# pranshu-raj-211/dmdqn

Measured on NVIDIA B200. Metric: agent-updates/sec, higher is better.
Workload: dtype f32

## Files before the change

dmdqn_b200/csrc/api.cu:

```cuda
#include <stdarg.h>
#include <string.h>
#include "common.cuh"

namespace dmdqn {

static thread_local char g_error[512] = "";

void set_error(const char* fmt, ...) {
    va_list ap;
    va_start(ap, fmt);
    vsnprintf(g_error, sizeof(g_error), fmt, ap);
    va_end(ap);
}

int validate_dims(const dmdqn_dims* d) {
    DMDQN_CHECK_ARG(d != nullptr, "dims is NULL");
    DMDQN_CHECK_ARG(d->n_agents >= 1, "n_agents=%d must be >= 1", d->n_agents);
    DMDQN_CHECK_ARG(d->n_nets == d->n_agents || d->n_nets == 1,
                    "n_nets=%d must be n_agents (independent) or 1 (shared)", d->n_nets);
    DMDQN_CHECK_ARG(d->obs_dim >= 1 && d->obs_stride >= d->obs_dim && d->obs_stride % 16 == 0 &&
                        d->obs_stride <= 128,
                    "obs_dim=%d obs_stride=%d: stride must be a multiple of 16 in [obs_dim, 128]",
                    d->obs_dim, d->obs_stride);
    DMDQN_CHECK_ARG(d->hidden == 64 || d->hidden == 128 || d->hidden == 256 || d->hidden == 512,
// ... 118 lines not shown
    if (rc) return rc;
    DMDQN_CHECK_ARG(nets && nets->theta && obs && eps && w_explore && w_action && actions_out, "act: NULL argument");
    DMDQN_CHECK_ARG(obs_in_stride >= dims->obs_dim, "obs_in_stride=%d < obs_dim=%d", obs_in_stride, dims->obs_dim);
    return launch_act(*dims, *nets, obs, obs_in_stride, eps, w_explore, w_action, actions_out, q_out, dueling,
                      (cudaStream_t)stream);
}

int dmdqn_act(const dmdqn_dims* dims, const dmdqn_nets* nets, const float* obs, int32_t obs_in_stride,
              const double* eps, const uint32_t* w_explore, const uint32_t* w_action, int32_t* actions_out,
              float* q_out, void* stream) {
    return run_act(dims, nets, obs, obs_in_stride, eps, w_explore, w_action, actions_out, q_out, false, stream);
}

int dmdqn_act_dueling(const dmdqn_dims* dims, const dmdqn_nets* nets, const float* obs, int32_t obs_in_stride,
                      const double* eps, const uint32_t* w_explore, const uint32_t* w_action, int32_t* actions_out,
                      float* q_out, void* stream) {
    return run_act(dims, nets, obs, obs_in_stride, eps, w_explore, w_action, actions_out, q_out, true, stream);
}

int dmdqn_push(const dmdqn_dims* dims, const dmdqn_replay* replay, const float* obs, const int32_t* act,
               const double* rew, const float* next_obs, const uint8_t* done, int32_t in_stride,
               const uint8_t* mask, void* stream) {
    int rc = validate_dims(dims);
    if (rc) return rc;
    DMDQN_CHECK_ARG(replay && replay->obs && replay->next_obs && replay->act && replay->rew && replay->done &&
                        replay->n_written, "push: NULL replay pointer");
    DMDQN_CHECK_ARG(!replay->priority || replay->priority_max, "push: priority is set but priority_max is NULL");
    DMDQN_CHECK_ARG(obs && act && rew && next_obs && done, "push: NULL transition pointer");
    DMDQN_CHECK_ARG(in_stride >= dims->obs_dim, "in_stride=%d < obs_dim=%d", in_stride, dims->obs_dim);
    return launch_push(*dims, *replay, obs, act, rew, next_obs, done, in_stride, mask, (cudaStream_t)stream);
}

static int check_n_step(const dmdqn_hparams* hp) {
    DMDQN_CHECK_ARG(hp->n_step >= 0 && hp->n_step <= DMDQN_MAX_NSTEP, "n_step=%d must be in [0, %d] (0 and 1: one-step targets)",
                    hp->n_step, DMDQN_MAX_NSTEP);
    return DMDQN_OK;
}

static_assert(offsetof(dmdqn_hparams, dueling) == 76 && sizeof(dmdqn_hparams) == 112,
              "dueling sits in the former interior padding of dmdqn_hparams: no other field moves");

static int check_dueling(const dmdqn_hparams* hp) {
    DMDQN_CHECK_ARG(hp->dueling == 0 || hp->dueling == 1, "dueling=%d must be 0 (plain head) or 1 (dueling heads)", hp->dueling);
    return DMDQN_OK;
}

static int check_learn_args(const dmdqn_dims* dims, const dmdqn_hparams* hp, const dmdqn_replay* replay,
                            const dmdqn_nets* nets, const void* draws) {
    DMDQN_CHECK_ARG(hp && replay && nets && draws, "NULL argument");
    if (int rc = check_n_step(hp)) return rc;
    if (int rc = check_dueling(hp)) return rc;
    DMDQN_CHECK_ARG(replay->obs && replay->next_obs && replay->act && replay->rew && replay->done &&
                        replay->n_written, "NULL replay pointer");
    DMDQN_CHECK_ARG(nets->theta && nets->theta_tgt && nets->adam_m && nets->adam_v && nets->learn_step,
                    "NULL network pointer");
    DMDQN_CHECK_ARG(hp->sample_mode >= 0 && hp->sample_mode <= DMDQN_SAMPLE_PRIORITIZED, "sample_mode=%d", hp->sample_mode);
    if (hp->sample_mode == DMDQN_SAMPLE_PRIORITIZED) {
        DMDQN_CHECK_ARG(replay->priority && replay->priority_max,
                        "sample_mode=prioritized needs the replay's priority and priority_max arrays (NULL priority pointer)");
        DMDQN_CHECK_ARG(!(dims->n_nets == 1 && dims->n_agents > 1),
                        "sample_mode=prioritized serves independent networks only (n_nets=%d, n_agents=%d share parameters)",
                        dims->n_nets, dims->n_agents);
    }
    DMDQN_CHECK_ARG(hp->loss == DMDQN_LOSS_MSE || hp->loss == DMDQN_LOSS_HUBER, "loss=%d", hp->loss);
    DMDQN_CHECK_ARG(hp->precision >= DMDQN_PRECISION_FP32 && hp->precision <= DMDQN_PRECISION_TF32X3, "precision=%d",
                    hp->precision);
    return DMDQN_OK;
}

static int run_learn(const dmdqn_dims* dims, const dmdqn_hparams* hp, const dmdqn_replay* replay, const dmdqn_nets* nets,
                     const void* draws, const uint8_t* learn_mask, float* metrics_out, void* workspace,
                     size_t workspace_bytes, int32_t stages, float* grads, int32_t global_batch, void* stream) {
    Workspace w;
    int rc = check_workspace(dims, workspace, workspace_bytes, &w);
    if (rc) return rc;
    rc = check_learn_args(dims, hp, replay, nets, draws);
    if (rc) return rc;
    if (grads) DMDQN_CHECK_ARG(global_batch >= dims->batch, "global_batch=%d < batch=%d", global_batch, dims->batch);
    if (stages & DMDQN_STAGE_SAMPLE) {
        if (hp->dueling) {
            rc = launch_fold(*dims, *nets, (char*)workspace, w, (cudaStream_t)stream);
            if (rc) return rc;
        }
        rc = launch_sample(*dims, *hp, *replay, *nets, draws, learn_mask, 1, (char*)workspace, w, (cudaStream_t)stream);
        if (rc) return rc;
    }
    return launch_learn(*dims, *hp, *replay, *nets, metrics_out, (char*)workspace, w, stages, grads, global_batch,
                        (cudaStream_t)stream);
}

int dmdqn_sample(const dmdqn_dims* dims, const dmdqn_hparams* hp, const dmdqn_replay* replay,
                 const dmdqn_nets* nets, const void* draws, const uint8_t* learn_mask, int32_t advance_step,
                 void* workspace, size_t workspace_bytes, void* stream) {
    Workspace w;
    int rc = check_workspace(dims, workspace, workspace_bytes, &w);
    if (rc) return rc;
    rc = check_learn_args(dims, hp, replay, nets, draws);
    if (rc) return rc;
    return launch_sample(*dims, *hp, *replay, *nets, draws, learn_mask, advance_step, (char*)workspace, w,
                         (cudaStream_t)stream);
}

int dmdqn_gather(const dmdqn_dims* dims, const dmdqn_replay* replay, const void* workspace,
                 size_t workspace_bytes, float* states, int32_t* actions, float* rewards, float* next_states,
                 float* dones, int32_t* active_out, void* stream) {
    Workspace w;
    int rc = check_workspace(dims, const_cast<void*>(workspace), workspace_bytes, &w);
    if (rc) return rc;
    DMDQN_CHECK_ARG(replay && replay->obs && replay->next_obs, "gather: NULL replay pointer");
    DMDQN_CHECK_ARG(states && actions && rewards && next_states && dones, "gather: NULL output");
    return launch_gather(*dims, *replay, (const char*)workspace, w, states, actions, rewards, next_states, dones,
                         active_out, (cudaStream_t)stream);
}

int dmdqn_learn_stages(const dmdqn_dims* dims, const dmdqn_hparams* hp, const dmdqn_replay* replay,
                       const dmdqn_nets* nets, const void* draws, const uint8_t* learn_mask, float* metrics_out,
                       void* workspace, size_t workspace_bytes, int32_t stages, void* stream) {
    return run_learn(dims, hp, replay, nets, draws, learn_mask, metrics_out, workspace, workspace_bytes, stages, nullptr, 0,
                     stream);
}

int dmdqn_learn(const dmdqn_dims* dims, const dmdqn_hparams* hp, const dmdqn_replay* replay,
                const dmdqn_nets* nets, const void* draws, const uint8_t* learn_mask, float* metrics_out,
                void* workspace, size_t workspace_bytes, void* stream) {
    return run_learn(dims, hp, replay, nets, draws, learn_mask, metrics_out, workspace, workspace_bytes, kAllStages, nullptr,
                     0, stream);
}

int dmdqn_step_host(const dmdqn_dims* dims, const dmdqn_hparams* hp, const dmdqn_replay* replay,
                    const dmdqn_nets* nets, const dmdqn_step_block* blk, const void* host_block, void* device_block,
                    float* metrics_dev, float* metrics_host, void* workspace, size_t workspace_bytes, void* stream) {
    int rc = validate_dims(dims);
    if (rc) return rc;
    DMDQN_CHECK_ARG(hp && blk && host_block && device_block && metrics_dev && metrics_host, "step_host: NULL argument");
    rc = check_n_step(hp);
    if (rc) return rc;
    rc = check_dueling(hp);
    if (rc) return rc;
    const size_t offs[6] = {blk->obs_off, blk->next_obs_off, blk->act_off, blk->rew_off, blk->done_off, blk->draws_off};
    for (size_t o : offs) DMDQN_CHECK_ARG(o % 16 == 0 && o < blk->bytes, "step_host: offset %zu is not a multiple of 16 inside the block", o);
    cudaStream_t s = (cudaStream_t)stream;
    char* d = static_cast<char*>(device_block);
    DMDQN_CUDA(cudaMemcpyAsync(d, host_block, blk->bytes, cudaMemcpyHostToDevice, s));
    rc = dmdqn_push(dims, replay, reinterpret_cast<const float*>(d + blk->obs_off), reinterpret_cast<const int32_t*>(d + blk->act_off),
                    reinterpret_cast<const double*>(d + blk->rew_off), reinterpret_cast<const float*>(d + blk->next_obs_off),
                    reinterpret_cast<const uint8_t*>(d + blk->done_off), blk->in_stride, nullptr, stream);
    if (rc) return rc;
    rc = dmdqn_learn(dims, hp, replay, nets, d + blk->draws_off, nullptr, metrics_dev, workspace, workspace_bytes, stream);
    if (rc) return rc;
    DMDQN_CUDA(cudaMemcpyAsync(metrics_host, metrics_dev, (size_t)dims->n_nets * DMDQN_METRICS_STRIDE * sizeof(float),
                               cudaMemcpyDeviceToHost, s));
    return DMDQN_OK;
}

int dmdqn_learn_grads(const dmdqn_dims* dims, const dmdqn_hparams* hp, const dmdqn_replay* replay,
                      const dmdqn_nets* nets, const void* draws, const uint8_t* learn_mask, int32_t global_batch,
                      float* grads_out, float* metrics_out, void* workspace, size_t workspace_bytes, void* stream) {
    DMDQN_CHECK_ARG(grads_out != nullptr, "grads_out is NULL");
    return run_learn(dims, hp, replay, nets, draws, learn_mask, metrics_out, workspace, workspace_bytes, kAllStages,
                     grads_out, global_batch, stream);
}

int dmdqn_adam_apply(const dmdqn_dims* dims, const dmdqn_hparams* hp, const dmdqn_nets* nets, const float* grads,
                     void* workspace, size_t workspace_bytes, void* stream) {
    Workspace w;
    int rc = check_workspace(dims, workspace, workspace_bytes, &w);
    if (rc) return rc;
// ... 239 lines not shown
```

dmdqn_b200/csrc/common.cuh:

```cuda
#pragma once
#include <cuda_runtime.h>
#include <stdint.h>
#include <stdio.h>
#include "../../include/dmdqn_b200.h"

namespace dmdqn {

void set_error(const char* fmt, ...);

#define DMDQN_CHECK_ARG(cond, ...)                                  \
    do {                                                            \
        if (!(cond)) {                                              \
            ::dmdqn::set_error(__VA_ARGS__);                        \
            return DMDQN_ERR_ARG;                                   \
        }                                                           \
    } while (0)

#define DMDQN_CUDA(expr)                                                              \
    do {                                                                              \
        cudaError_t _e = (expr);                                                      \
        if (_e != cudaSuccess) {                                                      \
            ::dmdqn::set_error("%s failed: %s", #expr, cudaGetErrorString(_e));       \
            return DMDQN_ERR_CUDA;                                                    \
        }                                                                             \
// ... 194 lines not shown
    float one_m_b1, one_m_b2, tau;
    int ws_tiles;
    int tc_tiles;
    const int32_t *rows, *nrows, *act_b, *active;
    const float *r_hat, *disc_b;
    const float4* adam_sc;
    float *y, *q_all, *q_next, *tq_all, *h1, *dh1, *dh2;
    float *part_loss, *part_b3, *part_w3, *part_b2, *part_b1;
    uint32_t* mask2;
    float2* ga;
    float* w3_copy;
    int* error;
    float* metrics;
    float* grads;
    int chain;
    int *sched, *k4a_done, *k3_done;
    int per;
    const float* is_w;
    double per_alpha, per_eps;
    const float* head[2];
    int64_t head_stride;
    int dueling;
};
LearnArgs make_learn_args(const dmdqn_dims& d, const dmdqn_hparams& hp, const dmdqn_replay& rp, const dmdqn_nets& nets,
                          char* ws, const Workspace& w, float* metrics, float* grads, int loss_batch);

__device__ __forceinline__ void per_store_priority(const LearnArgs& A, int row, float delta) {
    const float p = (float)pow(fabs((double)delta) + A.per_eps, A.per_alpha);
    if (!isfinite(p)) return;
    A.rp.priority[row] = p;
    atomicMax(reinterpret_cast<int*>(A.rp.priority_max) + row / A.d.capacity, __float_as_int(p));
}

struct AdamStep {
    float alpha, eps, one_m_b1, one_m_b2, tau;
    int sync;
};
__device__ __forceinline__ AdamStep adam_step(const LearnArgs& A, int g) {
    const float4 sc = __ldg(A.adam_sc + g);
    return {sc.x, sc.y, A.one_m_b1, A.one_m_b2, A.tau, __float_as_int(sc.z)};
}

template <typename Load>
__device__ __forceinline__ void finish_metrics(const LearnArgs& A, int g, int tiles, Load ld) {
    double ls = 0, qs = 0, qq = 0, hist[4] = {0, 0, 0, 0};
#pragma unroll 1
    for (int r = 0; r < tiles; ++r) {
        const float* pl = A.part_loss + ((size_t)g * tiles + r) * 8;
        ls += ld(pl); qs += ld(pl + 1); qq += ld(pl + 2);
        for (int a = 0; a < 4; ++a) hist[a] += ld(pl + 3 + a);
    }
    const double cnt = (double)A.d.batch * A.d.n_actions, mean = qs / cnt, var = fmax(qq / cnt - mean * mean, 0.0);
    float* m = A.metrics + g * DMDQN_METRICS_STRIDE;
    m[0] = (float)(ls / A.loss_batch);
    m[1] = (float)mean;
    m[2] = (float)sqrt(var);
    for (int a = 0; a < 4; ++a) m[3 + a] = (float)hist[a];
    m[7] = 1.f;
}

constexpr int kMaxDevices = 64;
int device_sm_count(int* n_sm);
int opt_in_dynamic_smem(const void* kernel, size_t bytes, size_t (&cache)[kMaxDevices]);

int launch_featurize(int32_t n, const int32_t* halting, const int32_t* phase, const double* next_switch,
                     const double* phase_dur, double sim_time, const uint8_t* signal_valid,
                     const int32_t* nbr_idx, const int32_t* phase_lut, const double* snapshot,
                     double lw, double gw, double* own_out, float* obs_out, int32_t obs_out_stride,
                     double* reward_out, double* global_out, int64_t* scratch, cudaStream_t s);
int launch_featurize_alt(int32_t n, const int32_t* halting, const int32_t* phase, const double* next_switch,
                         const uint8_t* signal_valid, double sim_time, const int32_t* nbr_idx, const double* prev_own,
                         double* own_out, float* obs_out, int32_t obs_out_stride, double* reward_out, cudaStream_t s);
int launch_act(const dmdqn_dims& d, const dmdqn_nets& nets, const float* obs, int32_t stride,
               const double* eps, const uint32_t* w1, const uint32_t* w2, int32_t* actions, float* q_out, bool dueling,
               cudaStream_t s, const dmdqn_noisy* noisy = nullptr);
int launch_noisy_fold(const dmdqn_dims& d, bool dueling, const dmdqn_nets& nets, const dmdqn_noisy& nz, cudaStream_t s);
int launch_noisy_adam_apply(const dmdqn_dims& d, const dmdqn_hparams& hp, const dmdqn_nets& nets, const dmdqn_noisy& nz,
                            const float* grads, char* ws, const Workspace& w, cudaStream_t s);
int launch_push(const dmdqn_dims& d, const dmdqn_replay& rp, const float* obs, const int32_t* act,
                const double* rew, const float* next_obs, const uint8_t* done, int32_t in_stride,
                const uint8_t* mask, cudaStream_t s);
int launch_sample(const dmdqn_dims& d, const dmdqn_hparams& hp, const dmdqn_replay& rp, const dmdqn_nets& nets,
                  const void* draws, const uint8_t* learn_mask, int advance, char* ws, const Workspace& w,
                  cudaStream_t s);
int launch_gather(const dmdqn_dims& d, const dmdqn_replay& rp, const char* ws, const Workspace& w,
                  float* states, int32_t* actions, float* rewards, float* next_states, float* dones,
                  int32_t* active_out, cudaStream_t s);
int launch_learn(const dmdqn_dims& d, const dmdqn_hparams& hp, const dmdqn_replay& rp, const dmdqn_nets& nets,
                 float* metrics, char* ws, const Workspace& w, int stages, float* grads, int loss_batch, cudaStream_t s);
bool tc_supported(const dmdqn_dims& d);
int launch_learn_tc(const LearnArgs& A, int precision, int stages, cudaStream_t s);
int launch_adam_apply(const dmdqn_dims& d, const dmdqn_hparams& hp, const dmdqn_nets& nets, const float* grads, char* ws,
                      const Workspace& w, cudaStream_t s);
int launch_clip_adam_apply(const dmdqn_dims& d, const dmdqn_hparams& hp, const dmdqn_nets& nets, const float* grads,
                           double clipnorm, float* norms_out, char* ws, const Workspace& w, cudaStream_t s);
int launch_sync_target(const dmdqn_dims& d, const dmdqn_nets& nets, const uint8_t* mask, double tau, bool dueling,
                       cudaStream_t s);
int launch_fold(const dmdqn_dims& d, const dmdqn_nets& nets, char* ws, const Workspace& w, cudaStream_t s);
int launch_peer_adam(const dmdqn_dims& d, const dmdqn_hparams& hp, const dmdqn_nets& nets, const dmdqn_peers& peers,
                     const float* my_loss_src, float* loss_out, char* ws, const Workspace& w, cudaStream_t s);

}
```

dmdqn_b200/csrc/learn_tc.cu:

```cuda
#include <cuda.h>
#include <string.h>
#include "common.cuh"

namespace dmdqn {

namespace {

constexpr int H = 256;
constexpr int BM = 128;
constexpr int EW = 16;
constexpr int NT = EW * 32;
constexpr int W_MMA = EW, W_TMA = EW + 1, W_CONV = EW + 2;
constexpr int CONV_WARPS = 6, CONV_GROUP_WARPS = 2;
constexpr int NT_F = (EW + 8) * 32;
constexpr int REGS_EPI = 104, REGS_AUX = 32;
constexpr int KC = 16;
constexpr uint32_t ATOM = BM * 128;
constexpr unsigned long long WAIT_LIMIT_NS = 2000000000ull;

__device__ __forceinline__ uint32_t smem_u32(const void* p) { return (uint32_t)__cvta_generic_to_shared(p); }

__device__ __forceinline__ uint64_t make_desc(uint32_t saddr, uint32_t lbo_bytes, uint32_t sbo_bytes, uint32_t layout) {
    return (uint64_t)((saddr >> 4) & 0x3FFF) | (uint64_t)((lbo_bytes >> 4) & 0x3FFF) << 16 |
           (uint64_t)((sbo_bytes >> 4) & 0x3FFF) << 32 | (uint64_t)1 << 46 | (uint64_t)layout << 61;
// ... 924 lines not shown
    th = th - __fdividef(m * k.alpha, sq + k.eps);
}

struct Wg {
    static constexpr int STAGES = 3;
    static constexpr uint32_t A_BYTES = KC * BM * 4;
    static constexpr uint32_t B_BYTES = KC * H * 4;
    static constexpr uint32_t AUX = 2 * A_BYTES + 2 * B_BYTES;
    static constexpr uint32_t AUX_MASK = 128;
    static constexpr uint32_t AUX_BYTES = 6144;
    static constexpr uint32_t STG = AUX + AUX_BYTES;
    static constexpr int TLD = 36;
    static constexpr uint32_t TILES = STAGES * STG;
    static constexpr uint32_t W3T = TILES + 8 * 32 * TLD * 4;
    static constexpr uint32_t BARS = W3T + 2 * 4 * H * 4;
    static constexpr uint32_t FULL = 0, CONV = 24, EMPTY = 48, ACC_FULL = 72, ACC_FREE = 88, TMEM = 104;
    static constexpr int NQ = 8;
    static constexpr uint32_t QFULL = 112, QITEM = QFULL + 8 * NQ;
    static constexpr uint32_t TOTAL = BARS + 256;
    static constexpr int EPI_WARPS = 8, CONV_WARPS = 8;
    static constexpr int NCONV = CONV_WARPS * 32;
    static constexpr int NTW = 20 * 32;
    static constexpr int REGS_EPI = 160, REGS_CONV = 64, REGS_AUX = 32;
};
__device__ __forceinline__ void conv_sync() { asm volatile("bar.sync 1, 256;" ::: "memory"); }

__device__ __forceinline__ void wg_item(int q, int G, int& g, int& t) {
    if (q < 2 * G) { g = q >> 1; t = q & 1; }
    else { g = q - 2 * G; t = 2; }
}

__device__ __forceinline__ int wg_pop(uint32_t bars, int& nq, bool& ok) {
    const uint32_t slot = (uint32_t)nq & (Wg::NQ - 1);
    int q = -1;
    if ((threadIdx.x & 31) == 0) {
        if (ok) ok = mbar_wait(bars + Wg::QFULL + 8 * slot, (uint32_t)(nq >> 3) & 1u);
        if (ok) asm volatile("ld.shared.s32 %0, [%1];" : "=r"(q) : "r"(bars + Wg::QITEM + 4 * slot));
    }
    ++nq;
    q = __shfl_sync(0xffffffffu, q, 0);
    if (q < 0) ok = __shfl_sync(0xffffffffu, (int)ok, 0) != 0;
    return q;
}
__device__ __forceinline__ float ldcg_f(const float* p) {
    float v;
    asm volatile("ld.global.cg.f32 %0, [%1];" : "=f"(v) : "l"(p));
    return v;
}

template <int PASSES>
__global__ void __launch_bounds__(Wg::NTW, 1) tc_wgrad_kernel(const LearnArgs A, const __grid_constant__ CUtensorMap tmap_h1,
                                                              const __grid_constant__ CUtensorMap tmap_dh1) {
    extern __shared__ uint8_t smem_raw[];
    const int B = A.d.batch, Dp = A.d.obs_stride, G = A.d.n_nets;
    const int tid = threadIdx.x, warp = tid >> 5, lane = tid & 31;
    const uint32_t sbase = (smem_u32(smem_raw) + 1023u) & ~1023u;
    const uint32_t bars = sbase + Wg::BARS;
    const int n_items = 3 * G;
    const int nchunks = (B + KC - 1) / KC;

    if (tid == 0) {
        for (int s = 0; s < Wg::STAGES; ++s) {
            mbar_init(bars + Wg::FULL + 8 * s, 1);
            mbar_init(bars + Wg::CONV + 8 * s, Wg::CONV_WARPS);
            mbar_init(bars + Wg::EMPTY + 8 * s, 1);
        }
        for (int b = 0; b < 2; ++b) {
            mbar_init(bars + Wg::ACC_FULL + 8 * b, 1);
            mbar_init(bars + Wg::ACC_FREE + 8 * b, Wg::EPI_WARPS);
        }
        for (int b = 0; b < Wg::NQ; ++b) mbar_init(bars + Wg::QFULL + 8 * b, 1);
        asm volatile("fence.mbarrier_init.release.cluster;" ::: "memory");
    }
    if (warp == 0) {
        asm volatile("tcgen05.alloc.cta_group::1.sync.aligned.shared::cta.b32 [%0], %1;" ::"r"(bars + Wg::TMEM), "r"(512));
        asm volatile("tcgen05.relinquish_alloc_permit.cta_group::1.sync.aligned;" ::);
    }
    tc_fence_before();
    __syncthreads();
    tc_fence_after();
    uint32_t tmem;
    asm volatile("ld.shared.u32 %0, [%1];" : "=r"(tmem) : "r"(bars + Wg::TMEM));
    bool ok = true;

    if (warp >= Wg::EPI_WARPS + Wg::CONV_WARPS) {
        regs_dec<Wg::REGS_AUX>();
        if (warp == Wg::EPI_WARPS + Wg::CONV_WARPS) {
            {
                uint32_t used = 0;
                int n = 0, nq = 0;
                for (;;) {
                    const int q = wg_pop(bars, nq, ok);
                    if (q < 0) break;
                    if (lane != 0) continue;
                    int g, t;
                    wg_item(q, G, g, t);
                    const bool is_w2 = t < 2;
                    const uint32_t acc_buf = (uint32_t)(n & 1);
                    const uint32_t d_tmem = tmem + acc_buf * 256u;
                    const uint32_t idesc = make_idesc(!is_w2, is_w2);
                    if (n >= 2 && ok)
                        ok = mbar_wait(bars + Wg::ACC_FREE + 8 * acc_buf, (uint32_t)((n >> 1) - 1) & 1u);
                    for (int c = 0; c < nchunks; ++c) {
                        const uint32_t s = used % Wg::STAGES, u = used / Wg::STAGES;
                        if (ok) ok = mbar_wait(bars + Wg::CONV + 8 * s, u & 1u);
                        tc_fence_after();
                        const uint32_t st = sbase + s * Wg::STG;
#pragma unroll
                        for (int ks = 0; ks < 2; ++ks) {
                            uint64_t a_hi, a_lo, b_hi, b_lo;
                            if (is_w2) {
                                a_hi = make_desc(st + ks * 32, 16, 512, 4);
                                a_lo = make_desc(st + Wg::A_BYTES + ks * 32, 16, 512, 4);
                                b_hi = make_desc(st + 2 * Wg::A_BYTES + ks * 2 * 4096, 512, 4096, 1);
                                b_lo = make_desc(st + 2 * Wg::A_BYTES + Wg::B_BYTES + ks * 2 * 4096, 512, 4096, 1);
                            } else {
                                a_hi = make_desc(st + ks * 2 * 2048, 512, 2048, 1);
                                a_lo = make_desc(st + Wg::A_BYTES + ks * 2 * 2048, 512, 2048, 1);
                                b_hi = make_desc(st + 2 * Wg::A_BYTES + ks * 32, 16, 512, 4);
                                b_lo = make_desc(st + 2 * Wg::A_BYTES + Wg::B_BYTES + ks * 32, 16, 512, 4);
                            }
                            uint32_t acc = (c | ks) ? 1u : 0u;
                            if (PASSES == 3) {
                                mma_ss(d_tmem, a_lo, b_hi, idesc, acc);
                                mma_ss(d_tmem, a_hi, b_lo, idesc, 1u);
                                acc = 1u;
                            }
                            mma_ss(d_tmem, a_hi, b_hi, idesc, acc);
                        }
                        umma_commit(bars + Wg::EMPTY + 8 * s);
                        if (c == nchunks - 1) umma_commit(bars + Wg::ACC_FULL + 8 * acc_buf);
                        ++used;
                    }
                    ++n;
                }
                if (!ok && lane == 0) atomicExch(A.error, 15);
            }
            __syncwarp();
        } else if (warp == Wg::EPI_WARPS + Wg::CONV_WARPS + 1) {
            uint32_t used = 0;
            int nq = 0;
            int draws = 0;
            for (;;) {
                int q = (int)blockIdx.x + draws * (int)gridDim.x;
                ++draws;
                if (A.chain) {
                    if (lane == 0) q = atomicAdd(A.sched, 1);
                    q = __shfl_sync(0xffffffffu, q, 0);
                }
                if (q >= n_items || !ok) break;
                int g, t;
                wg_item(q, G, g, t);
                if (!A.active[g]) {
                    if (t == 2 && lane < DMDQN_METRICS_STRIDE && A.metrics) A.metrics[g * DMDQN_METRICS_STRIDE + lane] = 0.f;
                    continue;
                }
                if (A.chain) {
                    int fine = 1;
                    if (lane == 0) {
                        fine = flag_acquire_ge(A.k4a_done + g, A.tc_tiles) ? 1 : 0;
                        asm volatile("fence.proxy.async;" ::: "memory");
                    }
                    ok = __shfl_sync(0xffffffffu, fine, 0) != 0;
                    if (!ok) break;
                }
                if (lane == 0) {
// ... 429 lines not shown
```

dmdqn_b200/csrc/replay.cu:

```cuda
#include "common.cuh"

namespace dmdqn {

namespace {

__global__ void __launch_bounds__(64)
push_kernel(dmdqn_dims d, dmdqn_replay rp, const float* __restrict__ obs, const int32_t* __restrict__ act,
            const double* __restrict__ rew, const float* __restrict__ next_obs,
            const uint8_t* __restrict__ done, int in_stride, const uint8_t* __restrict__ mask) {
    const int a = blockIdx.x;
    if (mask && !mask[a]) return;
    const long long nw = rp.n_written[a];
    const size_t row = (size_t)a * d.capacity + (size_t)(nw % d.capacity);
    float* dst_s = rp.obs + row * d.obs_stride;
    float* dst_n = rp.next_obs + row * d.obs_stride;
    for (int c = threadIdx.x; c < d.obs_stride; c += blockDim.x) {
        const bool in = c < d.obs_dim;
        dst_s[c] = in ? obs[(size_t)a * in_stride + c] : 0.f;
        dst_n[c] = in ? next_obs[(size_t)a * in_stride + c] : 0.f;
    }
    __syncthreads();
    if (threadIdx.x == 0) {
        rp.act[row] = act[a];
        rp.rew[row] = rew[a];
        rp.done[row] = done[a] ? 1 : 0;
        rp.n_written[a] = nw + 1;
        if (rp.priority) rp.priority[row] = rp.priority_max[a];
    }
}

constexpr int kSampleThreads = 256;
constexpr int kPerChunk = 128;
constexpr int kPerScan = 8;

template <typename F>
__device__ __forceinline__ double tree_sum(int n, int lane, F elem) {
    double acc = 0.0;
    for (int i = lane; i < n; i += 32) acc = __dadd_rn(acc, elem(i));
    for (int off = 16; off; off >>= 1) acc = __dadd_rn(acc, __shfl_xor_sync(0xffffffffu, acc, off));
    return acc;
}

__device__ __forceinline__ double nstep_return(const dmdqn_dims& d, const dmdqn_hparams& hp, const dmdqn_replay& rp, int row,
                                               int m, double z0, double mean, double denom, bool normalize) {
    if (m <= 1) return z0;
    const int C = d.capacity, agent = row / C, slot = row - agent * C;
    const double* rw = rp.rew + (size_t)agent * C;
    double r[DMDQN_MAX_NSTEP - 1];
#pragma unroll
    for (int k = 1; k < DMDQN_MAX_NSTEP; ++k) r[k - 1] = k < m ? rw[slot + k < C ? slot + k : slot + k - C] : 0.0;
    double ret = z0, gk = 1.0;
#pragma unroll
    for (int k = 1; k < DMDQN_MAX_NSTEP; ++k) {
        if (k < m) {
            gk = __dmul_rn(gk, hp.gamma);
            const double z = normalize ? __ddiv_rn(__dsub_rn(r[k - 1], mean), denom) : r[k - 1];
            ret = __dadd_rn(ret, __dmul_rn(gk, z));
        }
    }
    return ret;
}

template <bool PER, bool NSTEP>
__global__ void __launch_bounds__(kSampleThreads)
sample_kernel(dmdqn_dims d, dmdqn_hparams hp, dmdqn_replay rp, int32_t* __restrict__ learn_step,
              const uint32_t* __restrict__ draws, const uint8_t* __restrict__ learn_mask, int advance,
              int32_t* __restrict__ rows, float* __restrict__ r_hat, int32_t* __restrict__ act_b,
              float* __restrict__ done_b, int32_t* __restrict__ active, float4* __restrict__ adam_sc,
              int32_t* __restrict__ sync, int tiles, float* __restrict__ is_w, int32_t* __restrict__ nrows,
              float* __restrict__ disc_b) {
    extern __shared__ __align__(16) unsigned char smem_raw[];
    const int B = d.batch, Bp = (B + 1) & ~1;
    int* js = reinterpret_cast<int*>(smem_raw);
    int* pt = js + Bp;
    int* words = pt + Bp;
    double* rs = reinterpret_cast<double*>(words + Bp);
    __shared__ double stat[2];
    __shared__ int per_last, per_pmin;
    __shared__ double per_beta;
    const int g = blockIdx.x, tid = threadIdx.x, lane = tid & 31;
    const bool per = hp.sample_mode == DMDQN_SAMPLE_PRIORITIZED;
    const bool shared_net = d.n_nets == 1 && d.n_agents > 1;
    asm volatile("griddepcontrol.launch_dependents;" ::: "memory");
    if (tid < 4 && g == 0) sync[tid] = 0;
    if (tid == 4) sync[4 + g] = 0;
    if (tid >= 32 && tid < 32 + tiles) sync[4 + d.n_nets + g * tiles + (tid - 32)] = 0;

    const long long nw0 = rp.n_written[shared_net ? 0 : g];
    const int size0 = (int)(nw0 < d.capacity ? nw0 : d.capacity);
    const long long pop = shared_net ? (long long)size0 * d.n_agents : size0;
    const bool on = (learn_mask == nullptr || learn_mask[g]) && pop >= B;
    int t_step = 0;
    if (tid == 0) {
        active[g] = on ? 1 : 0;
        int t = learn_step[g];
        if (on && advance) learn_step[g] = ++t;
        t_step = t;
    }
    if (!on) return;
    auto adam_scalars = [&]() {
        const int t = t_step;
        const double bc1 = 1.0 - pow(hp.beta1, (double)t), bc2 = 1.0 - pow(hp.beta2, (double)t);
        const int freq = hp.target_update_frequency > 0 ? hp.target_update_frequency : 1;
        const int sync_mode = hp.tau >= 0.0 ? 2 : (t % freq == 0 ? 1 : 0);
        adam_sc[g] = make_float4((float)(hp.learning_rate * sqrt(bc2) / bc1),
                                 (float)(hp.adam_form == DMDQN_ADAM_KERAS ? hp.adam_eps : hp.adam_eps * sqrt(bc2)),
                                 __int_as_float(sync_mode), 0.f);
    };

    if constexpr (PER) {
        const int C = d.capacity, nch = (C + kPerChunk - 1) / kPerChunk, warp = tid >> 5;
        const float* __restrict__ pr = rp.priority + (size_t)g * C;
        double* prefix = rs + Bp;
        if (tid == 0) { per_last = -1; per_pmin = 0x7f800000; }
        int last = -1;
        for (int c0 = warp * kPerScan; c0 < nch; c0 += (kSampleThreads / 32) * kPerScan) {
            float v[kPerScan][4];
#pragma unroll
            for (int u = 0; u < kPerScan; ++u)
#pragma unroll
                for (int k = 0; k < 4; ++k) {
                    const int sl = (c0 + u) * kPerChunk + 32 * k + lane;
                    v[u][k] = sl < C ? __ldg(pr + sl) : 0.f;
                }
#pragma unroll
            for (int u = 0; u < kPerScan; ++u) {
                double acc = 0.0;
#pragma unroll
                for (int k = 0; k < 4; ++k) {
                    acc = __dadd_rn(acc, (double)v[u][k]);
                    if (v[u][k] > 0.f) last = (c0 + u) * kPerChunk + 32 * k + lane;
                }
                for (int off = 16; off; off >>= 1) acc = __dadd_rn(acc, __shfl_xor_sync(0xffffffffu, acc, off));
                if (lane == 0 && c0 + u < nch) prefix[c0 + u + 1] = acc;
            }
        }
        last = __reduce_max_sync(0xffffffffu, last);
        __syncthreads();
        if (lane == 0 && last >= 0) atomicMax(&per_last, last);
        if (tid == 32) {
            double run = 0.0;
            prefix[0] = 0.0;
            for (int c = 1; c <= nch; ++c) {
                run = __dadd_rn(run, prefix[c]);
                prefix[c] = run;
            }
        }
        if (tid == 0) {
            adam_scalars();
            double beta = hp.per_beta0;
            if (hp.per_beta_steps > 0)
                beta = fmin(1.0, __dadd_rn(hp.per_beta0, __ddiv_rn(__dmul_rn(__dsub_rn(1.0, hp.per_beta0), (double)t_step),
                                                                   (double)hp.per_beta_steps)));
            per_beta = beta;
        }
        __syncthreads();
        const double S = prefix[nch];
        for (int i = tid; i < B; i += kSampleThreads) {
            const double w = (double)draws[(size_t)g * B + i];
            const double u = __ddiv_rn(__dmul_rn(__dadd_rn((double)i, __dmul_rn(w, 0x1p-32)), S), (double)B);
            int lo = 0, hi = nch - 1;
            while (lo < hi) {
                const int mid = (lo + hi + 1) >> 1;
                if (prefix[mid] <= u) lo = mid; else hi = mid - 1;
            }
            const int base = lo * kPerChunk;
            double run = prefix[lo];
            int slot = -1;
            for (int s0 = 0; s0 < kPerChunk && slot < 0; s0 += 32) {
                float v[32];
#pragma unroll
                for (int k = 0; k < 32; ++k) v[k] = base + s0 + k < C ? __ldg(pr + base + s0 + k) : 0.f;
#pragma unroll
                for (int k = 0; k < 32; ++k) {
                    run = __dadd_rn(run, (double)v[k]);
                    if (slot < 0 && run > u) slot = base + s0 + k;
                }
            }
            if (slot < 0) slot = per_last >= 0 ? per_last : 0;
            words[i] = slot;
            atomicMin(&per_pmin, __float_as_int(__ldg(pr + slot)));
        }
    } else if (hp.sample_mode == DMDQN_SAMPLE_FISHER_YATES) {
        const int n = (int)pop;
        for (int i = tid; i < B; i += kSampleThreads)
            js[i] = (int)__umulhi(draws[(size_t)g * B + i], (unsigned)(n - i));
        __syncthreads();
        for (int i0 = 0; i0 < B; i0 += kSampleThreads) {
            const int i = i0 + tid;
            const int ji = i < B ? js[i] : -1, ti = i < B ? n - i - 1 : -1;
            int pj = -1, ptk = -1;
            const int kend = min(B, i0 + (tid | 31));
#pragma unroll 4
            for (int k = 0; k < kend; ++k) {
                const int jk = js[k];
                const bool before = k < i;
                pj = (before && jk == ji) ? k : pj;
                ptk = (before && jk == ti) ? k : ptk;
            }
            if (i < B) { pt[i] = ptk; words[i] = pj; }
        }
        if (tid == 0) adam_scalars();
        __syncthreads();
        for (int i = tid; i < B; i += kSampleThreads) {
            int k = words[i];
            int v = js[i];
            if (k >= 0) {
                while (pt[k] >= 0) k = pt[k];
                v = n - k - 1;
            }
            words[i] = v;
        }
    } else if (hp.sample_mode == DMDQN_SAMPLE_REPLACEMENT) {
        for (int i = tid; i < B; i += kSampleThreads) words[i] = (int)__umulhi(draws[(size_t)g * B + i], (unsigned)pop);
        if (tid == 0) adam_scalars();
    } else {
        for (int i = tid; i < B; i += kSampleThreads) {
            const int v = (int)draws[(size_t)g * B + i];
            words[i] = v < 0 ? 0 : (v >= pop ? (int)pop - 1 : v);
        }
        if (tid == 0) adam_scalars();
    }
    __syncthreads();

    for (int i = tid; i < B; i += kSampleThreads) {
        const int logical = words[i];
        const int agent = shared_net ? logical / size0 : g;
        const int lj = shared_net ? logical % size0 : logical;
        const long long nw = shared_net ? rp.n_written[agent] : nw0;
        const long long sz = nw < d.capacity ? nw : d.capacity;
        const int slot = per ? words[i] : (int)((nw - sz + lj) % d.capacity);
        const int row = agent * d.capacity + slot;
        if constexpr (PER) {
            const float p = rp.priority[row];
            is_w[(size_t)g * B + i] = p > 0.f ? (float)pow(__ddiv_rn((double)__int_as_float(per_pmin), (double)p), per_beta) : 1.f;
        }
        rows[(size_t)g * B + i] = row;
        act_b[(size_t)g * B + i] = rp.act[row];
        if constexpr (!NSTEP) {
            const bool dn = rp.done[row];
            done_b[(size_t)g * B + i] = dn ? 1.f : 0.f;
            js[i] = row;
            pt[i] = dn;
        }
        rs[i] = rp.rew[row];
        if constexpr (NSTEP) {
            const int C = d.capacity;
            const int j = per ? (int)(((long long)slot - (nw - sz) % C + C) % C) : lj;
            const int lim = min(hp.n_step, (int)sz - j);
            const uint8_t* dn = rp.done + (size_t)agent * C;
            unsigned bits = 0;
#pragma unroll
            for (int k = 0; k < DMDQN_MAX_NSTEP; ++k)
                if (k < lim && dn[slot + k < C ? slot + k : slot + k - C]) bits |= 1u << k;
            const int m = bits ? __ffs(bits) : lim;
            double gm = hp.gamma;
            for (int k = 1; k < m; ++k) gm = __dmul_rn(gm, hp.gamma);
            const int last = slot + m - 1;
            nrows[(size_t)g * B + i] = agent * C + (last < C ? last : last - C);
            done_b[(size_t)g * B + i] = bits ? 1.f : 0.f;
            disc_b[(size_t)g * B + i] = bits ? 0.f : (float)gm;
            js[i] = row;
            pt[i] = m;
        }
    }
    __syncthreads();
    if constexpr (!NSTEP) {
        for (int i = tid - 32; tid >= 32 && i < B; i += kSampleThreads - 32) {
            nrows[(size_t)g * B + i] = js[i];
            disc_b[(size_t)g * B + i] = (float)hp.gamma * (1.0f - (pt[i] ? 1.f : 0.f));
        }
    }
    if (hp.normalize_rewards) {
        if (tid < 32) {
            const double mean = __ddiv_rn(tree_sum(B, lane, [&](int i) { return rs[i]; }), (double)B);
            const double var = __ddiv_rn(tree_sum(B, lane, [&](int i) {
                                             const double dv = __dsub_rn(rs[i], mean);
                                             return __dmul_rn(dv, dv);
                                         }), (double)B);
            if (lane == 0) { stat[0] = mean; stat[1] = __dadd_rn(__dsqrt_rn(var), 1e-8); }
        }
        __syncthreads();
        const double mean = stat[0], denom = stat[1];
        for (int i = tid; i < B; i += kSampleThreads) {
            const double z = __ddiv_rn(__dsub_rn(rs[i], mean), denom);
            r_hat[(size_t)g * B + i] = (float)(NSTEP ? nstep_return(d, hp, rp, js[i], pt[i], z, mean, denom, true) : z);
        }
    } else {
        for (int i = tid; i < B; i += kSampleThreads)
            r_hat[(size_t)g * B + i] = (float)(NSTEP ? nstep_return(d, hp, rp, js[i], pt[i], rs[i], 0.0, 1.0, false) : rs[i]);
    }
}

__global__ void __launch_bounds__(128)
gather_kernel(dmdqn_dims d, dmdqn_replay rp, const int32_t* __restrict__ rows, const int32_t* __restrict__ nrows,
              const float* __restrict__ r_hat,
              const int32_t* __restrict__ act_b, const float* __restrict__ done_b,
              const int32_t* __restrict__ active, float* __restrict__ states, int32_t* __restrict__ actions,
              float* __restrict__ rewards, float* __restrict__ next_states, float* __restrict__ dones,
              int32_t* __restrict__ active_out) {
    const int lane = threadIdx.x & 31;
    const long long r = (long long)blockIdx.x * 4 + (threadIdx.x >> 5);
    const long long total = (long long)d.n_nets * d.batch;
    if (r >= total) return;
    const int g = (int)(r / d.batch);
    if (active_out && (r % d.batch) == 0 && lane == 0) active_out[g] = active[g];
    if (!active[g]) return;
    const size_t src = (size_t)rows[r] * d.obs_stride;
    const size_t nsrc = (size_t)nrows[r] * d.obs_stride;
    const int q = d.obs_stride >> 2;
    float4 s4 = make_float4(0.f, 0.f, 0.f, 0.f), n4 = s4;
    if (lane < q) {
        s4 = __ldg(reinterpret_cast<const float4*>(rp.obs + src) + lane);
        n4 = __ldg(reinterpret_cast<const float4*>(rp.next_obs + nsrc) + lane);
    }
#pragma unroll
    for (int k = 0; k < 4; ++k) {
        const int c = 32 * k + lane, from = 8 * k + (lane >> 2);
        const float sx = __shfl_sync(0xffffffffu, s4.x, from), sy = __shfl_sync(0xffffffffu, s4.y, from);
        const float sz = __shfl_sync(0xffffffffu, s4.z, from), sw = __shfl_sync(0xffffffffu, s4.w, from);
        const float nx = __shfl_sync(0xffffffffu, n4.x, from), ny = __shfl_sync(0xffffffffu, n4.y, from);
        const float nz = __shfl_sync(0xffffffffu, n4.z, from), nw = __shfl_sync(0xffffffffu, n4.w, from);
        const int comp = lane & 3;
        if (c < d.obs_dim) {
            states[r * d.obs_dim + c] = comp == 0 ? sx : comp == 1 ? sy : comp == 2 ? sz : sw;
            next_states[r * d.obs_dim + c] = comp == 0 ? nx : comp == 1 ? ny : comp == 2 ? nz : nw;
        }
    }
    if (lane == 0) {
        actions[r] = act_b[r];
        rewards[r] = r_hat[r];
        dones[r] = done_b[r];
    }
}

}

int launch_push(const dmdqn_dims& d, const dmdqn_replay& rp, const float* obs, const int32_t* act,
                const double* rew, const float* next_obs, const uint8_t* done, int32_t in_stride,
                const uint8_t* mask, cudaStream_t s) {
    push_kernel<<<d.n_agents, 64, 0, s>>>(d, rp, obs, act, rew, next_obs, done, in_stride, mask);
    DMDQN_CUDA(cudaGetLastError());
    return DMDQN_OK;
}

int launch_sample(const dmdqn_dims& d, const dmdqn_hparams& hp, const dmdqn_replay& rp, const dmdqn_nets& nets,
                  const void* draws, const uint8_t* learn_mask, int advance, char* ws, const Workspace& w,
                  cudaStream_t s) {
    DMDQN_CHECK_ARG(d.batch <= 4096, "batch %d: the sample kernel serves batches up to 4096", d.batch);
    const bool per = hp.sample_mode == DMDQN_SAMPLE_PRIORITIZED;
    DMDQN_CHECK_ARG(!per || d.capacity <= DMDQN_PER_MAX_CAPACITY,
                    "capacity=%d: prioritized replay serves rings of up to %d slots", d.capacity, DMDQN_PER_MAX_CAPACITY);
    const size_t smem = (size_t)((d.batch + 1) & ~1) * (3 * 4 + 8) +
                        (per ? (size_t)((d.capacity + kPerChunk - 1) / kPerChunk + 1) * 8 : 0);
    const bool nstep = hp.n_step > 1;
    static size_t configured[4][kMaxDevices] = {};
    const auto kernel = per ? (nstep ? sample_kernel<true, true> : sample_kernel<true, false>)
                            : (nstep ? sample_kernel<false, true> : sample_kernel<false, false>);
    if (int rc = opt_in_dynamic_smem(reinterpret_cast<const void*>(kernel), smem, configured[2 * per + nstep])) return rc;
    kernel<<<d.n_nets, kSampleThreads, smem, s>>>(
        d, hp, rp, nets.learn_step, static_cast<const uint32_t*>(draws), learn_mask, advance,
        reinterpret_cast<int32_t*>(ws + w.rows), reinterpret_cast<float*>(ws + w.r_hat),
        reinterpret_cast<int32_t*>(ws + w.act_b), reinterpret_cast<float*>(ws + w.done_b),
        reinterpret_cast<int32_t*>(ws + w.active), reinterpret_cast<float4*>(ws + w.adam_sc),
        reinterpret_cast<int32_t*>(ws + w.sync), w.tiles, reinterpret_cast<float*>(ws + w.is_w),
        reinterpret_cast<int32_t*>(ws + w.nrows), reinterpret_cast<float*>(ws + w.disc_b));
    DMDQN_CUDA(cudaGetLastError());
    return DMDQN_OK;
}

int launch_gather(const dmdqn_dims& d, const dmdqn_replay& rp, const char* ws, const Workspace& w,
                  float* states, int32_t* actions, float* rewards, float* next_states, float* dones,
                  int32_t* active_out, cudaStream_t s) {
    const long long total = (long long)d.n_nets * d.batch;
    gather_kernel<<<(unsigned)((total + 3) / 4), 128, 0, s>>>(
        d, rp, reinterpret_cast<const int32_t*>(ws + w.rows), reinterpret_cast<const int32_t*>(ws + w.nrows),
        reinterpret_cast<const float*>(ws + w.r_hat),
        reinterpret_cast<const int32_t*>(ws + w.act_b), reinterpret_cast<const float*>(ws + w.done_b),
        reinterpret_cast<const int32_t*>(ws + w.active), states, actions, rewards, next_states, dones,
        active_out);
    DMDQN_CUDA(cudaGetLastError());
    return DMDQN_OK;
}

}
```

Before: 541,200.

## Chain sample kernel into tensor-core learn via programmatic dependent launch

Launches the sample kernel with programmatic stream serialization when it directly feeds the tensor-core learn path. The kernel now stages its outputs in shared memory and writes them to global only after griddepcontrol.wait. This lets the sampling work overlap the tail of the previous learn kernel, and the learn kernel now triggers dependents early. It adds shared memory per block and a staging pass, and it relies on careful wait placement for correctness.

```diff
diff --git a/dmdqn_b200/csrc/api.cu b/dmdqn_b200/csrc/api.cu
--- a/dmdqn_b200/csrc/api.cu
+++ b/dmdqn_b200/csrc/api.cu
@@ -224,7 +224,9 @@
             rc = launch_fold(*dims, *nets, (char*)workspace, w, (cudaStream_t)stream);
             if (rc) return rc;
         }
-        rc = launch_sample(*dims, *hp, *replay, *nets, draws, learn_mask, 1, (char*)workspace, w, (cudaStream_t)stream);
+        const bool chained = stages == kAllStages && hp->precision != DMDQN_PRECISION_FP32 && tc_supported(*dims);
+        rc = launch_sample(*dims, *hp, *replay, *nets, draws, learn_mask, 1, (char*)workspace, w, (cudaStream_t)stream,
+                           chained);
         if (rc) return rc;
     }
     return launch_learn(*dims, *hp, *replay, *nets, metrics_out, (char*)workspace, w, stages, grads, global_batch,
diff --git a/dmdqn_b200/csrc/common.cuh b/dmdqn_b200/csrc/common.cuh
--- a/dmdqn_b200/csrc/common.cuh
+++ b/dmdqn_b200/csrc/common.cuh
@@ -300,7 +300,7 @@
                 const uint8_t* mask, cudaStream_t s);
 int launch_sample(const dmdqn_dims& d, const dmdqn_hparams& hp, const dmdqn_replay& rp, const dmdqn_nets& nets,
                   const void* draws, const uint8_t* learn_mask, int advance, char* ws, const Workspace& w,
-                  cudaStream_t s);
+                  cudaStream_t s, bool chained = false);
 int launch_gather(const dmdqn_dims& d, const dmdqn_replay& rp, const char* ws, const Workspace& w,
                   float* states, int32_t* actions, float* rewards, float* next_states, float* dones,
                   int32_t* active_out, cudaStream_t s);
diff --git a/dmdqn_b200/csrc/learn_tc.cu b/dmdqn_b200/csrc/learn_tc.cu
--- a/dmdqn_b200/csrc/learn_tc.cu
+++ b/dmdqn_b200/csrc/learn_tc.cu
@@ -1030,6 +1030,7 @@
     uint32_t tmem;
     asm volatile("ld.shared.u32 %0, [%1];" : "=r"(tmem) : "r"(bars + Wg::TMEM));
     bool ok = true;
+    if (A.chain) pdl_launch_dependents();
 
     if (warp >= Wg::EPI_WARPS + Wg::CONV_WARPS) {
         regs_dec<Wg::REGS_AUX>();
diff --git a/dmdqn_b200/csrc/replay.cu b/dmdqn_b200/csrc/replay.cu
--- a/dmdqn_b200/csrc/replay.cu
+++ b/dmdqn_b200/csrc/replay.cu
@@ -68,7 +68,7 @@
               int32_t* __restrict__ rows, float* __restrict__ r_hat, int32_t* __restrict__ act_b,
               float* __restrict__ done_b, int32_t* __restrict__ active, float4* __restrict__ adam_sc,
               int32_t* __restrict__ sync, int tiles, float* __restrict__ is_w, int32_t* __restrict__ nrows,
-              float* __restrict__ disc_b) {
+              float* __restrict__ disc_b, int chained) {
     extern __shared__ __align__(16) unsigned char smem_raw[];
     const int B = d.batch, Bp = (B + 1) & ~1;
     int* js = reinterpret_cast<int*>(smem_raw);
@@ -81,10 +81,8 @@
     const int g = blockIdx.x, tid = threadIdx.x, lane = tid & 31;
     const bool per = hp.sample_mode == DMDQN_SAMPLE_PRIORITIZED;
     const bool shared_net = d.n_nets == 1 && d.n_agents > 1;
-    asm volatile("griddepcontrol.launch_dependents;" ::: "memory");
-    if (tid < 4 && g == 0) sync[tid] = 0;
-    if (tid == 4) sync[4 + g] = 0;
-    if (tid >= 32 && tid < 32 + tiles) sync[4 + d.n_nets + g * tiles + (tid - 32)] = 0;
+    if (chained) asm volatile("griddepcontrol.launch_dependents;" ::: "memory");
+    if constexpr (PER) asm volatile("griddepcontrol.wait;" ::: "memory");
 
     const long long nw0 = rp.n_written[shared_net ? 0 : g];
     const int size0 = (int)(nw0 < d.capacity ? nw0 : d.capacity);
@@ -92,20 +90,33 @@
     const bool on = (learn_mask == nullptr || learn_mask[g]) && pop >= B;
     int t_step = 0;
     if (tid == 0) {
-        active[g] = on ? 1 : 0;
-        int t = learn_step[g];
-        if (on && advance) learn_step[g] = ++t;
-        t_step = t;
-    }
-    if (!on) return;
+        t_step = learn_step[g];
+        if (on && advance) ++t_step;
+    }
+    float4 sc = make_float4(0.f, 0.f, 0.f, 0.f);
+    auto publish = [&]() {
+        asm volatile("griddepcontrol.wait;" ::: "memory");
+        if (tid < 4 && g == 0) sync[tid] = 0;
+        if (tid == 4) sync[4 + g] = 0;
+        if (tid >= 32 && tid < 32 + tiles) sync[4 + d.n_nets + g * tiles + (tid - 32)] = 0;
+        if (tid == 0) {
+            active[g] = on ? 1 : 0;
+            if (on && advance) learn_step[g] = t_step;
+            if (on) adam_sc[g] = sc;
+        }
+    };
+    if (!on) {
+        publish();
+        return;
+    }
     auto adam_scalars = [&]() {
         const int t = t_step;
         const double bc1 = 1.0 - pow(hp.beta1, (double)t), bc2 = 1.0 - pow(hp.beta2, (double)t);
         const int freq = hp.target_update_frequency > 0 ? hp.target_update_frequency : 1;
         const int sync_mode = hp.tau >= 0.0 ? 2 : (t % freq == 0 ? 1 : 0);
-        adam_sc[g] = make_float4((float)(hp.learning_rate * sqrt(bc2) / bc1),
-                                 (float)(hp.adam_form == DMDQN_ADAM_KERAS ? hp.adam_eps : hp.adam_eps * sqrt(bc2)),
-                                 __int_as_float(sync_mode), 0.f);
+        sc = make_float4((float)(hp.learning_rate * sqrt(bc2) / bc1),
+                         (float)(hp.adam_form == DMDQN_ADAM_KERAS ? hp.adam_eps : hp.adam_eps * sqrt(bc2)),
+                         __int_as_float(sync_mode), 0.f);
     };
 
     if constexpr (PER) {
@@ -223,6 +234,7 @@
     }
     __syncthreads();
 
+    float* out = reinterpret_cast<float*>(rs + Bp + (PER ? (d.capacity + kPerChunk - 1) / kPerChunk + 1 : 0));
     for (int i = tid; i < B; i += kSampleThreads) {
         const int logical = words[i];
         const int agent = shared_net ? logical / size0 : g;
@@ -233,13 +245,12 @@
         const int row = agent * d.capacity + slot;
         if constexpr (PER) {
             const float p = rp.priority[row];
-            is_w[(size_t)g * B + i] = p > 0.f ? (float)pow(__ddiv_rn((double)__int_as_float(per_pmin), (double)p), per_beta) : 1.f;
-        }
-        rows[(size_t)g * B + i] = row;
-        act_b[(size_t)g * B + i] = rp.act[row];
+            out[Bp + i] = p > 0.f ? (float)pow(__ddiv_rn((double)__int_as_float(per_pmin), (double)p), per_beta) : 1.f;
+        }
+        words[i] = rp.act[row];
         if constexpr (!NSTEP) {
             const bool dn = rp.done[row];
-            done_b[(size_t)g * B + i] = dn ? 1.f : 0.f;
+            out[i] = dn ? 1.f : 0.f;
             js[i] = row;
             pt[i] = dn;
         }
@@ -257,20 +268,14 @@
             double gm = hp.gamma;
             for (int k = 1; k < m; ++k) gm = __dmul_rn(gm, hp.gamma);
             const int last = slot + m - 1;
-            nrows[(size_t)g * B + i] = agent * C + (last < C ? last : last - C);
-            done_b[(size_t)g * B + i] = bits ? 1.f : 0.f;
-            disc_b[(size_t)g * B + i] = bits ? 0.f : (float)gm;
+            out[2 * Bp + i] = __int_as_float(agent * C + (last < C ? last : last - C));
+            out[i] = bits ? 1.f : 0.f;
+            out[3 * Bp + i] = bits ? 0.f : (float)gm;
             js[i] = row;
             pt[i] = m;
         }
     }
     __syncthreads();
-    if constexpr (!NSTEP) {
-        for (int i = tid - 32; tid >= 32 && i < B; i += kSampleThreads - 32) {
-            nrows[(size_t)g * B + i] = js[i];
-            disc_b[(size_t)g * B + i] = (float)hp.gamma * (1.0f - (pt[i] ? 1.f : 0.f));
-        }
-    }
     if (hp.normalize_rewards) {
         if (tid < 32) {
             const double mean = __ddiv_rn(tree_sum(B, lane, [&](int i) { return rs[i]; }), (double)B);
@@ -284,11 +289,28 @@
         const double mean = stat[0], denom = stat[1];
         for (int i = tid; i < B; i += kSampleThreads) {
             const double z = __ddiv_rn(__dsub_rn(rs[i], mean), denom);
-            r_hat[(size_t)g * B + i] = (float)(NSTEP ? nstep_return(d, hp, rp, js[i], pt[i], z, mean, denom, true) : z);
+            out[4 * Bp + i] = (float)(NSTEP ? nstep_return(d, hp, rp, js[i], pt[i], z, mean, denom, true) : z);
         }
     } else {
         for (int i = tid; i < B; i += kSampleThreads)
-            r_hat[(size_t)g * B + i] = (float)(NSTEP ? nstep_return(d, hp, rp, js[i], pt[i], rs[i], 0.0, 1.0, false) : rs[i]);
+            out[4 * Bp + i] = (float)(NSTEP ? nstep_return(d, hp, rp, js[i], pt[i], rs[i], 0.0, 1.0, false) : rs[i]);
+    }
+
+    publish();
+    for (int i = tid; i < B; i += kSampleThreads) {
+        const size_t o = (size_t)g * B + i;
+        rows[o] = js[i];
+        act_b[o] = words[i];
+        done_b[o] = out[i];
+        if constexpr (PER) is_w[o] = out[Bp + i];
+        if constexpr (NSTEP) {
+            nrows[o] = __float_as_int(out[2 * Bp + i]);
+            disc_b[o] = out[3 * Bp + i];
+        } else {
+            nrows[o] = js[i];
+            disc_b[o] = (float)hp.gamma * (1.0f - (pt[i] ? 1.f : 0.f));
+        }
+        r_hat[o] = out[4 * Bp + i];
     }
 }
 
@@ -346,26 +368,35 @@
 
 int launch_sample(const dmdqn_dims& d, const dmdqn_hparams& hp, const dmdqn_replay& rp, const dmdqn_nets& nets,
                   const void* draws, const uint8_t* learn_mask, int advance, char* ws, const Workspace& w,
-                  cudaStream_t s) {
+                  cudaStream_t s, bool chained) {
     DMDQN_CHECK_ARG(d.batch <= 4096, "batch %d: the sample kernel serves batches up to 4096", d.batch);
     const bool per = hp.sample_mode == DMDQN_SAMPLE_PRIORITIZED;
     DMDQN_CHECK_ARG(!per || d.capacity <= DMDQN_PER_MAX_CAPACITY,
                     "capacity=%d: prioritized replay serves rings of up to %d slots", d.capacity, DMDQN_PER_MAX_CAPACITY);
-    const size_t smem = (size_t)((d.batch + 1) & ~1) * (3 * 4 + 8) +
+    const size_t smem = (size_t)((d.batch + 1) & ~1) * (3 * 4 + 8 + 5 * 4) +
                         (per ? (size_t)((d.capacity + kPerChunk - 1) / kPerChunk + 1) * 8 : 0);
     const bool nstep = hp.n_step > 1;
     static size_t configured[4][kMaxDevices] = {};
     const auto kernel = per ? (nstep ? sample_kernel<true, true> : sample_kernel<true, false>)
                             : (nstep ? sample_kernel<false, true> : sample_kernel<false, false>);
     if (int rc = opt_in_dynamic_smem(reinterpret_cast<const void*>(kernel), smem, configured[2 * per + nstep])) return rc;
-    kernel<<<d.n_nets, kSampleThreads, smem, s>>>(
-        d, hp, rp, nets.learn_step, static_cast<const uint32_t*>(draws), learn_mask, advance,
+    cudaLaunchAttribute pdl[1];
+    pdl[0].id = cudaLaunchAttributeProgrammaticStreamSerialization;
+    pdl[0].val.programmaticStreamSerializationAllowed = 1;
+    cudaLaunchConfig_t cfg = {};
+    cfg.gridDim = dim3(d.n_nets);
+    cfg.blockDim = dim3(kSampleThreads);
+    cfg.dynamicSmemBytes = smem;
+    cfg.stream = s;
+    cfg.attrs = pdl;
+    cfg.numAttrs = chained ? 1 : 0;
+    DMDQN_CUDA(cudaLaunchKernelEx(
+        &cfg, kernel, d, hp, rp, nets.learn_step, static_cast<const uint32_t*>(draws), learn_mask, advance,
         reinterpret_cast<int32_t*>(ws + w.rows), reinterpret_cast<float*>(ws + w.r_hat),
         reinterpret_cast<int32_t*>(ws + w.act_b), reinterpret_cast<float*>(ws + w.done_b),
         reinterpret_cast<int32_t*>(ws + w.active), reinterpret_cast<float4*>(ws + w.adam_sc),
         reinterpret_cast<int32_t*>(ws + w.sync), w.tiles, reinterpret_cast<float*>(ws + w.is_w),
-        reinterpret_cast<int32_t*>(ws + w.nrows), reinterpret_cast<float*>(ws + w.disc_b));
-    DMDQN_CUDA(cudaGetLastError());
+        reinterpret_cast<int32_t*>(ws + w.nrows), reinterpret_cast<float*>(ws + w.disc_b), (int)chained));
     return DMDQN_OK;
 }
 
```

New measurement: 557,800 (median of 6 runs). 1.03x the previous value.
